# faasm/faabric

Measured on AMD Instinct MI355X. Metric: MPI_Allreduce GB/s + batch-exec msgs/sec, 8-rank world at 1/2/4/8 MI355X, higher is better.
Workload: dtype fp32; 1 GPU; model=faabric composite: 256MB fp32 allreduce + 1MB alltoall + kvtouch batch, global_batch=128, parallelism=mpi1, allreduce_bytes=268435456, pingpong_bytes=0, kv_bytes=4096, full=False, snapshot_bytes_per_rank=0, snapshot_dirty=random-scattered 25pct, random-byte region, gpu=True

## Files before the change

cpp/bindings/bindings_runtime.cpp:

```cpp
#include <pybind11/functional.h>
#include <pybind11/pybind11.h>
#include <pybind11/stl.h>

#include "faabricamd/endpoint.h"
#include "faabricamd/executor.h"
#include "faabricamd/flat.h"
#include "faabricamd/hipipc.h"
#include "faabricamd/planner.h"
#include "faabricamd/ptp.h"
#include "faabricamd/runner.h"
#include "faabricamd/scheduler.h"
#include "faabricamd/snapshot.h"
#include "faabricamd/state.h"
#include "faabricamd/util.h"
#include "faabricamd/utilextras.h"
#include "faabricamd/dirty.h"
#include <hip/hip_runtime.h>

namespace py = pybind11;
using namespace faabricamd;

namespace faabricamd {
void registerBenchFunctions();
std::map<std::string, std::vector<uint8_t>> benchLastOutputs();
// ... 826 lines not shown
            ok = dirty.size() == 16 && dirty[5] == 1 && dirty[12] == 1;
        }
        return py::bool_(ok);
    });

    m.def("_debug_runtime_sizes", [] {
        py::dict d;
        d["planner_app_results"] = Planner::get().debugAppResultsCount();
        d["planner_done_apps"] = Planner::get().debugDoneAppsCount();
        d["planner_in_flight"] = Planner::get().debugInFlightCount();
        d["broker_mappings"] = getPointToPointBroker().debugMappingsCount();
        d["broker_channels"] = getPointToPointBroker().debugChannelsCount();
        d["broker_send_seqs"] = getPointToPointBroker().debugSendSeqsCount();
        d["decision_cache"] = DecisionCache::get().size();
        return d;
    });
    m.def("_debug_dispatch_sizes", [] {
        py::dict d;
        d["idle_executors"] = Scheduler::get().debugIdleCount();
        d["planner_msg_index_apps"] = Planner::get().debugMsgIndexCount();
        d["planner_used_slots"] = Planner::get().debugUsedSlots();
        return d;
    });
    m.def("_debug_current_executor_id", [] {
        return ExecutorContext::get().getExecutor()->id;
    });
    m.def("_debug_set_message_result", [](const Message& msg) {
        auto copy = std::make_shared<Message>(msg);
        py::gil_scoped_release release;
        getPlannerClient().setMessageResult(copy);
    });
    m.def("_debug_kv_commit_stats", [] {
        KvCommitStats s = kvCommitStats();
        py::dict d;
        d["launches"] = s.launches;
        d["pages"] = s.pages;
        return d;
    });
    m.def("_debug_kv_sweep_bitmap",
          [](size_t nPages, const std::vector<uint64_t>& setBits) {
              size_t nWords = (nPages + 63) / 64;
              auto words = std::make_unique<std::atomic<uint64_t>[]>(
                std::max<size_t>(nWords, 1));
              for (size_t w = 0; w < nWords; w++) {
                  words[w].store(0);
              }
// ... 203 lines not shown
```

cpp/include/faabricamd/executor.h:

```cpp
#pragma once

#include <atomic>
#include <functional>
#include <memory>
#include <string>
#include <thread>
#include <vector>

#include "faabricamd/mailbox.h"
#include "faabricamd/messages.h"
#include "faabricamd/queue.h"
#include "faabricamd/dirty.h"
#include "faabricamd/snapshot.h"

namespace faabricamd {

class Executor;


class ExecutorContext
{
  public:
    static bool isSet();
    static void set(Executor* executor,
                    std::shared_ptr<BatchExecuteRequest> req,
                    int msgIdx);
    static void unset();
// ... 5 lines not shown
        return req;
    }
    Message& getMsg();
    int getMsgIdx() const { return msgIdx; }

  private:
    Executor* executor = nullptr;
    std::shared_ptr<BatchExecuteRequest> req;
    int msgIdx = 0;
};


using FaabricFunction = std::function<int32_t(Message&)>;

class FunctionRegistry
{
  public:
    static FunctionRegistry& get();
    void registerFunction(const std::string& user,
                          const std::string& function,
                          FaabricFunction fn);
    FaabricFunction* getFunction(const std::string& user,
                                 const std::string& function);
    void clear();

  private:
    std::mutex mx;
    std::map<std::string, FaabricFunction> functions;
};


struct ExecutorTask
{
    ExecutorTask() = default;
    ExecutorTask(int msgIdxIn, std::shared_ptr<BatchExecuteRequest> reqIn)
      : msgIdx(msgIdxIn)
      , req(std::move(reqIn))
    {}
    int msgIdx = 0;
    std::shared_ptr<BatchExecuteRequest> req;
    bool stop = false;
    bool single = false;
    int64_t enqueueNs = 0;
};

class Executor : public std::enable_shared_from_this<Executor>
{
  public:
    explicit Executor(Message& msg);
    virtual ~Executor();

    void executeTasks(const std::vector<int>& msgIdxs,
                      const std::shared_ptr<BatchExecuteRequest>& req);
    void executeSingleTask(int msgIdx,
                           const std::shared_ptr<BatchExecuteRequest>& req);

    std::vector<std::pair<int32_t, int32_t>> executeThreads(
      std::shared_ptr<BatchExecuteRequest> req,
      const std::vector<SnapshotMergeRegion>& mergeRegions);

    virtual int32_t executeTask(int threadPoolIdx,
                                int msgIdx,
                                std::shared_ptr<BatchExecuteRequest> req);

    virtual std::pair<uint8_t*, size_t> getMemoryView();
    virtual void setMemorySize(size_t newSize);
    void setDeviceMemorySize(size_t newSize);
    std::pair<uint8_t*, size_t> getDeviceMemoryView();
    bool hasDeviceArena() const { return deviceArena != nullptr; }
    virtual void restore(const std::string& snapshotKey);
    virtual void reset(Message& msg);
    virtual void flush();

    bool tryClaim();
    void claim();
    void releaseClaim();
    bool isClaimed() const { return claimed.load(); }
    using IdleExecutors = IdleList<std::shared_ptr<Executor>>;
// ... 73 lines not shown
```

cpp/include/faabricamd/mailbox.h:

```cpp
#pragma once

#include <atomic>
#include <climits>
#include <cstddef>
#include <cstdint>
#include <ctime>
#include <mutex>
#include <utility>
#include <vector>

#include <linux/futex.h>
#include <sys/syscall.h>
#include <unistd.h>

namespace faabricamd {

namespace detail {

inline void futexWait(std::atomic<uint32_t>* word,
                      uint32_t expected,
                      int timeoutMs)
{
    static_assert(sizeof(std::atomic<uint32_t>) == sizeof(uint32_t));
    struct timespec ts;
    struct timespec* tsp = nullptr;
    if (timeoutMs > 0) {
        ts.tv_sec = timeoutMs / 1000;
        ts.tv_nsec = (long)(timeoutMs % 1000) * 1000000L;
        tsp = &ts;
// ... 18 lines not shown
            0);
}

}

template<typename T, uint32_t SLOTS = 8>
class Mailbox
{
    static_assert(SLOTS >= 2 && (SLOTS & (SLOTS - 1)) == 0,
                  "SLOTS must be a power of two");

  public:
    Mailbox()
    {
        for (uint32_t i = 0; i < SLOTS; i++) {
            slots[i].seq.store(i, std::memory_order_relaxed);
        }
    }
    Mailbox(const Mailbox&) = delete;
    Mailbox& operator=(const Mailbox&) = delete;

    void post(T value)
    {
        uint32_t ticket = tail.fetch_add(1, std::memory_order_relaxed);
        Slot& s = slots[ticket & (SLOTS - 1)];
        uint32_t seen;
        while ((seen = s.seq.load(std::memory_order_acquire)) != ticket) {
            detail::futexWait(&s.seq, seen, 1);
        }
        s.value = std::move(value);
        s.seq.store(ticket + 1, std::memory_order_seq_cst);
        if (sleeping.load(std::memory_order_seq_cst) != 0) {
            detail::futexWake(&s.seq, INT_MAX);
        }
    }

    bool take(T& out, int timeoutMs)
    {
        Slot& s = slots[head & (SLOTS - 1)];
        uint32_t ready = head + 1;
        uint32_t seen = s.seq.load(std::memory_order_acquire);
        if (seen != ready) {
            struct timespec start;
            clock_gettime(CLOCK_MONOTONIC, &start);
            int leftMs = timeoutMs;
            while (true) {
                sleeping.store(1, std::memory_order_seq_cst);
                seen = s.seq.load(std::memory_order_seq_cst);
                if (seen != ready) {
                    detail::futexWait(&s.seq, seen, leftMs);
                    seen = s.seq.load(std::memory_order_acquire);
                }
                sleeping.store(0, std::memory_order_relaxed);
                if (seen == ready) {
                    break;
                }
                if (timeoutMs > 0) {
                    struct timespec now;
                    clock_gettime(CLOCK_MONOTONIC, &now);
                    int64_t goneMs =
                      (int64_t)(now.tv_sec - start.tv_sec) * 1000 +
                      (now.tv_nsec - start.tv_nsec) / 1000000;
                    if (goneMs >= timeoutMs) {
                        return false;
                    }
                    leftMs = (int)(timeoutMs - goneMs);
                }
            }
        }
        out = std::move(s.value);
        s.value = T();
        s.seq.store(head + SLOTS, std::memory_order_release);
        head++;
        return true;
    }

  private:
    struct alignas(64) Slot
    {
        std::atomic<uint32_t> seq{ 0 };
        T value{};
    };
    Slot slots[SLOTS];
    alignas(64) std::atomic<uint32_t> tail{ 0 };
    std::atomic<uint32_t> sleeping{ 0 };
    alignas(64) uint32_t head = 0;
};

template<typename T>
class IdleList
{
  public:
    void push(T value)
    {
        std::lock_guard<std::mutex> lock(mx);
        if (!closed) {
            entries.push_back(std::move(value));
        }
    }

    size_t popMany(size_t n, std::vector<T>& out)
    {
        std::lock_guard<std::mutex> lock(mx);
        size_t got = 0;
        while (got < n && !entries.empty()) {
            out.push_back(std::move(entries.back()));
            entries.pop_back();
            got++;
        }
        return got;
    }
// ... 53 lines not shown
```

cpp/include/faabricamd/scheduler.h:

```cpp
#pragma once

#include <memory>
#include <mutex>
#include <shared_mutex>
#include <unordered_map>
#include <vector>

#include "faabricamd/executor.h"
#include "faabricamd/messages.h"
#include "faabricamd/queue.h"
#include "faabricamd/transport.h"

namespace faabricamd {

enum class FunctionCalls : uint8_t
{
    ExecuteFunctions = 1,
    Flush = 2,
    SetMessageResult = 3,
    BatchDone = 4,
};

class Scheduler
{
// ... 3 lines not shown
    void executeBatch(std::shared_ptr<BatchExecuteRequest> req);

    HostResources getThisHostResources();
    void setThisHostResources(const HostResources& res);

    int reapStaleExecutors();
    void startReaper();
    void stopReaper();

    std::shared_ptr<PendingMigration> checkForMigrationOpportunities(
      Message& msg,
      int32_t overwriteNewGroupId = 0);

    void flushLocally();
    void shutdown();
    void reset();

    std::vector<Message> getRecordedMessages();
    void clearRecordedMessages();

    size_t getExecutorCount();
    size_t debugIdleCount();

  private:
    Scheduler();

    struct WarmPool
    {
        std::vector<std::shared_ptr<Executor>> list;
        std::shared_ptr<Executor::IdleExecutors> idle =
          std::make_shared<Executor::IdleExecutors>();
    };

    std::shared_ptr<Executor> claimExecutor(Message& msg);
    void claimExecutors(BatchExecuteRequest& req,
                        std::vector<std::shared_ptr<Executor>>& execs,
                        std::vector<std::string>& errors);
    std::shared_ptr<Executor> createExecutorLocked(WarmPool& pool,
                                                   Message& msg);

    std::shared_mutex schedMx;
    std::unordered_map<std::string, std::unique_ptr<WarmPool>> executors;
    HostResources overriddenResources;
    bool resourcesOverridden = false;

    std::vector<Message> recordedMessages;

    class ReaperThread;
    std::shared_ptr<ReaperThread> reaper;
};

bool functionCallServerRunning();

class FunctionCallServer : public MessageEndpointServer
{
  public:
    FunctionCallServer();
    ~FunctionCallServer() override;
// ... 30 lines not shown
```

cpp/include/faabricamd/state.h:

```cpp
#pragma once

#include <atomic>
#include <map>
#include <memory>
#include <mutex>
#include <string>
#include <vector>

#include "faabricamd/hipipc.h"
#include "faabricamd/messages.h"
#include "faabricamd/transport.h"

namespace faabricamd {

inline constexpr size_t STATE_STREAM_CHUNK_SIZE = 64 * 1024;

enum class StateCalls : uint8_t
{
    Pull = 1,
    Push = 2,
    Size = 3,
    Append = 4,
    ClearAppended = 5,
    PullAppended = 6,
    Delete = 7,
    PullIpc = 8,
    PushIpc = 9,
    Lock = 10,
// ... 135 lines not shown
    void forceClearAll(bool global);
    void syncAll();

    uint64_t acquireLock(const std::string& user,
                         const std::string& key,
                         int expiryMs);
    void releaseLock(const std::string& user,
                     const std::string& key,
                     uint64_t token);
    uint64_t acquireLockLocal(const std::string& user,
                              const std::string& key,
                              int expiryMs);
    bool releaseLockLocal(const std::string& user,
                          const std::string& key,
                          uint64_t token);

    void setMasterHost(const std::string& user,
                       const std::string& key,
                       const std::string& host);
    std::string getMasterHost(const std::string& user,
                              const std::string& key);

  private:
    std::mutex mx;
    std::map<std::string, std::shared_ptr<StateKeyValue>> kvMap;
    std::map<std::string, std::string> masterMap;

    std::mutex locksMx;
    std::map<std::string, std::pair<uint64_t, int64_t>> locks;
};

class StateServer : public MessageEndpointServer
{
  public:
    StateServer();
    void doAsyncRecv(uint8_t code,
                     const std::string& body,
                     uint32_t seq) override;
    std::string doSyncRecv(uint8_t code, const std::string& body) override;
};

class StateClient : public MessageEndpointClient
{
  public:
    explicit StateClient(const std::string& host);
    std::vector<uint8_t> pullChunk(const std::string& user,
                                   const std::string& key,
// ... 37 lines not shown
```

cpp/include/faabricamd/utilextras.h:

```cpp
#pragma once

#include <cstdint>
#include <string>
#include <vector>

namespace faabricamd {


struct DeltaConfig
{
    size_t pageSize = 4096;
    bool xorWithOld = true;
    bool compress = true;
    bool useZstd = true;

    static DeltaConfig parse(const std::string& s);
    std::string str() const;
};

std::vector<uint8_t> deltaEncode(const std::vector<uint8_t>& oldData,
                                 const std::vector<uint8_t>& newData,
                                 const DeltaConfig& conf = {});

std::vector<uint8_t> deltaApply(const std::vector<uint8_t>& oldData,
                                const std::vector<uint8_t>& delta);


void profStart(const std::string& name);
void profEnd(const std::string& name);
bool profEnabled();
int64_t profNowNs();
void profRecord(const char* name, double ms);
std::vector<std::pair<std::string, double>> profTotalsMs();
void profClear();
std::string profSummary();

#define PROF_START(name)                                                       \
    if (::faabricamd::profEnabled()) {                                         \
        ::faabricamd::profStart(#name);                                        \
    }
#define PROF_END(name)                                                         \
    if (::faabricamd::profEnabled()) {                                         \
        ::faabricamd::profEnd(#name);                                          \
    }

class ProfScope
{
  public:
    explicit ProfScope(const char* nameIn)
      : name(nameIn)
      , startNs(profEnabled() ? profNowNs() : 0)
    {}
    ~ProfScope()
    {
        if (startNs != 0) {
            profRecord(name, (double)(profNowNs() - startNs) / 1e6);
        }
    }
    ProfScope(const ProfScope&) = delete;
    ProfScope& operator=(const ProfScope&) = delete;

  private:
    const char* name;
    int64_t startNs;
};

void setUpCrashHandler();

int pinThreadToFreeCpu();
void unpinThisThread();

}
```

cpp/src/executor.cpp:

```cpp
#include "faabricamd/executor.h"
#include "faabricamd/utilextras.h"
#include "faabricamd/mpi.h"
#include "faabricamd/ops.h"
#include "faabricamd/planner.h"

#include <hip/hip_runtime.h>
#include "faabricamd/snapshot.h"
#include "faabricamd/util.h"

#include <algorithm>
#include <cstring>

namespace faabricamd {

void resultBatcherEnqueue(std::shared_ptr<Message> msg);


static thread_local std::shared_ptr<ExecutorContext> currentContext;

bool ExecutorContext::isSet()
{
    return currentContext != nullptr;
}

// ... 17 lines not shown
{
    if (!currentContext) {
        throw FaabricException("no executor context set");
    }
    return *currentContext;
}

Message& ExecutorContext::getMsg()
{
    return req->messages.at(msgIdx);
}


FunctionRegistry& FunctionRegistry::get()
{
    static FunctionRegistry reg;
    return reg;
}

void FunctionRegistry::registerFunction(const std::string& user,
                                        const std::string& function,
                                        FaabricFunction fn)
{
    std::lock_guard<std::mutex> lock(mx);
    functions[user + "/" + function] = std::move(fn);
}

FaabricFunction* FunctionRegistry::getFunction(const std::string& user,
                                               const std::string& function)
{
    std::lock_guard<std::mutex> lock(mx);
    auto it = functions.find(user + "/" + function);
    return it == functions.end() ? nullptr : &it->second;
}

void FunctionRegistry::clear()
{
    std::lock_guard<std::mutex> lock(mx);
    functions.clear();
}


Executor::Executor(Message& msg)
  : id(funcToString(msg.user, msg.function, 0) + "_" +
       std::to_string(generateGid()))
  , boundMsg(msg)
{
    threadPoolSize = std::min(getUsableCores(), 64);
    threadMailboxes.resize(threadPoolSize);
    threadPoolThreads.resize(threadPoolSize);
    poolThreadUp = std::make_unique<std::atomic<bool>[]>(threadPoolSize);
    for (int i = 0; i < threadPoolSize; i++) {
        poolThreadUp[i].store(false, std::memory_order_relaxed);
    }
    lastExecMs = getGlobalClockEpochMillis();
}

void Executor::cleanupForkSnapshot()
{
    if (lastForkSnapshotKey.empty()) {
        return;
    }
// ... 101 lines not shown
void Executor::ensurePoolThreadLocked(int poolIdx)
{
    if (threadPoolThreads[poolIdx].joinable()) {
        return;
    }
    if (!threadMailboxes[poolIdx]) {
        threadMailboxes[poolIdx] = std::make_unique<TaskMailbox>();
    }
    threadPoolThreads[poolIdx] =
      std::thread([this, poolIdx] { threadPoolThread(poolIdx); });
    poolThreadUp[poolIdx].store(true, std::memory_order_release);
}

void Executor::postTask(int poolIdx, ExecutorTask&& task)
{
    task.enqueueNs = profEnabled() ? profNowNs() : 0;
    threadMailboxes[poolIdx]->post(std::move(task));
}

void Executor::executeSingleTask(
  int msgIdx,
  const std::shared_ptr<BatchExecuteRequest>& req)
{
    if (req->type == BatchExecuteType::THREADS ||
        !req->snapshotKey.empty() ||
        !req->messages.at(msgIdx).snapshotKey.empty() ||
        threadPoolSize == 0) {
        executeTasks({ msgIdx }, req);
        return;
    }
    lastExecMs = getGlobalClockEpochMillis();
    if (!poolThreadUp[0].load(std::memory_order_acquire)) {
        std::lock_guard<std::mutex> lock(threadsMx);
        ensurePoolThreadLocked(0);
    }
    ExecutorTask task(msgIdx, req);
    task.single = true;
    postTask(0, std::move(task));
}

void Executor::executeTasks(const std::vector<int>& msgIdxs,
                            const std::shared_ptr<BatchExecuteRequest>& req)
{
    lastExecMs = getGlobalClockEpochMillis();
    batchCounter = std::make_shared<std::atomic<int>>((int)msgIdxs.size());

    if (!req->snapshotKey.empty()) {
        restore(req->snapshotKey);
    } else if (!req->messages.empty() &&
               !req->messages[msgIdxs[0]].snapshotKey.empty() &&
               req->type != BatchExecuteType::THREADS) {
        const std::string& key = req->messages[msgIdxs[0]].snapshotKey;
        restore(key);
        if (startsWith(key, "migration_")) {
            SnapshotRegistry::get().deleteSnapshot(key);
            DeviceSnapshotRegistry::get().deleteSnapshot(key);
        }
    }

    if (req->type == BatchExecuteType::THREADS &&
        !req->snapshotKey.empty()) {
// ... 128 lines not shown
        hipError_t err = hipMemcpy(deviceArena,
                                   dsnap->data(),
                                   dsnap->size(),
                                   hipMemcpyDeviceToDevice);
        if (err != hipSuccess ||
            hipStreamSynchronize(nullptr) != hipSuccess) {
            throw FaabricException("device snapshot merge-back failed");
        }
    } else {
        snap->writeQueuedDiffs();
        auto [memBase2, memSize2] = getMemoryView();
        snap->mapToMemory(memBase2, memSize2);
        snap->clearMergeRegions();
    }
    return results;
}

int32_t Executor::executeTask(int threadPoolIdx,
                              int msgIdx,
                              std::shared_ptr<BatchExecuteRequest> req)
{
    (void)threadPoolIdx;
    Message& msg = req->messages.at(msgIdx);
    FaabricFunction* fn =
      FunctionRegistry::get().getFunction(msg.user, msg.function);
    if (fn == nullptr) {
        throw FaabricException("function not registered: " + msg.user + "/" +
                               msg.function);
    }
    return (*fn)(msg);
}

std::pair<uint8_t*, size_t> Executor::getMemoryView()
{
    return { dummyMemory.data(), dummyMemory.size() };
}

void Executor::setMemorySize(size_t newSize)
{
    dummyMemory.resize(newSize);
}

void Executor::restore(const std::string& snapshotKey)
{
    const auto& conf = getSystemConfig();
    int64_t deadline = getGlobalClockEpochMillis() + conf.boundTimeout;
    while (true) {
        if (DeviceSnapshotRegistry::get().snapshotExists(snapshotKey)) {
            auto dsnap =
              DeviceSnapshotRegistry::get().getSnapshot(snapshotKey);
            if (deviceArenaSize < dsnap->size()) {
                setDeviceMemorySize(dsnap->size());
            }
// ... 36 lines not shown
void Executor::setThreadResult(Message& msg,
                               int32_t returnValue,
                               const std::string& key,
                               const std::vector<SnapshotDiffMsg>& diffs)
{
    (void)key;
    (void)diffs;
    msg.returnValue = returnValue;
}

void Executor::threadPoolThread(int poolIdx)
{
    const auto& conf = getSystemConfig();
    TaskMailbox& mailbox = *threadMailboxes[poolIdx];
    while (true) {
        ExecutorTask task;
        if (!mailbox.take(task, conf.boundTimeout)) {
            continue;
        }
        if (task.stop) {
            break;
        }
        if (task.enqueueNs != 0) {
            profRecord("exec_wake",
                       (double)(profNowNs() - task.enqueueNs) / 1e6);
        }

        Message& msg = task.req->messages.at(task.msgIdx);
        int32_t returnValue = 0;
        ExecutorContext::set(this, task.req, task.msgIdx);
        try {
            PROF_START(exec_task)
            returnValue = executeTask(poolIdx, task.msgIdx, task.req);
            PROF_END(exec_task)
            if (msg.isMpi && msg.recordExecGraph &&
                MpiWorldRegistry::get().worldExists(msg.mpiWorldId)) {
                auto counts = MpiWorldRegistry::get()
                                .getWorld(msg.mpiWorldId)
                                .getMsgCountDetails(msg.mpiRank);
                for (const auto& [k, v] : counts) {
                    msg.intExecGraphDetails[k] = v;
                }
            }
        } catch (const FunctionMigratedException&) {
            FAM_DEBUG("task %d migrated", msg.id);
            returnValue = MIGRATED_FUNCTION_RETURN_VALUE;
        } catch (const FunctionFrozenException&) {
            FAM_DEBUG("task %d frozen", msg.id);
// ... 259 lines not shown
```

cpp/src/scheduler.cpp:

```cpp
#include "faabricamd/scheduler.h"
#include "faabricamd/utilextras.h"

#include <atomic>
#include <thread>
#include <functional>
#include <condition_variable>
#include "faabricamd/planner.h"
#include "faabricamd/ptp.h"
#include "faabricamd/util.h"
#include "faabricamd/wire.h"

#include <hip/hip_runtime.h>

namespace faabricamd {

static int getNumGpus()
{
    static int n = []() {
        const auto& conf = getSystemConfig();
        if (conf.overrideGpuCount >= 0) {
            return conf.overrideGpuCount;
        }
        if (!conf.useGpu) {
            return 0;
// ... 23 lines not shown

HostResources Scheduler::getThisHostResources()
{
    {
        std::unique_lock<std::shared_mutex> lock(schedMx);
        if (resourcesOverridden) {
            return overriddenResources;
        }
    }
    HostResources res;
    int nGpus = getNumGpus();
    res.slots = nGpus > 0 ? nGpus : getUsableCores();
    res.usedSlots = 0;
    return res;
}

void Scheduler::setThisHostResources(const HostResources& res)
{
    std::unique_lock<std::shared_mutex> lock(schedMx);
    overriddenResources = res;
    resourcesOverridden = true;
}

void Scheduler::executeBatch(std::shared_ptr<BatchExecuteRequest> req)
{
    if (req->messages.empty()) {
        return;
    }
    PROF_START(sched_execute_batch)
    bool isThreads = req->type == BatchExecuteType::THREADS;

    if (isTestMode()) {
        std::unique_lock<std::shared_mutex> lock(schedMx);
        for (const auto& msg : req->messages) {
            recordedMessages.push_back(msg);
        }
    }

    if (isThreads) {
        auto exec = claimExecutor(req->messages[0]);
        std::vector<int> idxs(req->messages.size());
        for (size_t i = 0; i < idxs.size(); i++) {
            idxs[i] = (int)i;
        }
        exec->executeTasks(idxs, req);
    } else {
        size_t n = req->messages.size();
        std::vector<std::shared_ptr<Executor>> execs;
        std::vector<std::string> claimErrors;
        PROF_START(dispatch_claim)
        claimExecutors(*req, execs, claimErrors);
        PROF_END(dispatch_claim)

        PROF_START(dispatch_enqueue)
        for (size_t i = 0; i < n; i++) {
            try {
                if (!execs[i]) {
                    throw FaabricException(claimErrors[i]);
                }
                execs[i]->executeSingleTask((int)i, req);
            } catch (const std::exception& e) {
                FAM_ERROR("claiming executor failed: %s", e.what());
                if (execs[i]) {
                    execs[i]->releaseClaim();
                }
                auto msg = std::make_shared<Message>(req->messages[i]);
                msg->returnValue = 1;
                msg->executedHost = getSystemConfig().endpointHost;
                msg->outputData = std::string("executor claim failed: ") +
                                  e.what();
                getPlannerClient().setMessageResult(msg);
            }
        }
        PROF_END(dispatch_enqueue)
    }
    PROF_END(sched_execute_batch)
}

static std::shared_ptr<Executor> popIdleClaimed(
  Executor::IdleExecutors& idle)
{
    std::shared_ptr<Executor> e;
    while (idle.pop(e)) {
        if (e->tryClaim()) {
            return e;
        }
    }
    return nullptr;
}

std::shared_ptr<Executor> Scheduler::createExecutorLocked(WarmPool& pool,
                                                          Message& msg)
{
    auto exec = getExecutorFactory()->createExecutor(msg);
    exec->claim();
// ... 14 lines not shown
    std::string key = msg.user + "/" + msg.function;

    {
        std::shared_lock<std::shared_mutex> rlock(schedMx);
        auto it = executors.find(key);
        if (it != executors.end()) {
            if (auto e = popIdleClaimed(*it->second->idle)) {
                return e;
            }
        }
    }

    std::unique_lock<std::shared_mutex> lock(schedMx);
    auto& poolPtr = executors[key];
    if (!poolPtr) {
        poolPtr = std::make_unique<WarmPool>();
    }
    if (auto e = popIdleClaimed(*poolPtr->idle)) {
        return e;
    }
    return createExecutorLocked(*poolPtr, msg);
}

void Scheduler::claimExecutors(
  BatchExecuteRequest& req,
  std::vector<std::shared_ptr<Executor>>& execs,
  std::vector<std::string>& errors)
{
    size_t n = req.messages.size();
    execs.assign(n, nullptr);
    errors.assign(n, std::string());

    const Message& first = req.messages[0];
    bool oneFunction = true;
    for (size_t i = 1; i < n && oneFunction; i++) {
        oneFunction = req.messages[i].function == first.function &&
                      req.messages[i].user == first.user;
    }
    if (!oneFunction) {
        for (size_t i = 0; i < n; i++) {
            try {
                execs[i] = claimExecutor(req.messages[i]);
            } catch (const std::exception& e) {
                errors[i] = e.what();
            }
        }
        return;
    }

    std::string key = first.user + "/" + first.function;
    std::vector<std::shared_ptr<Executor>> popped;
    popped.reserve(n);
    size_t got = 0;
    auto takeIdle = [&](Executor::IdleExecutors& idle) {
        while (got < n) {
            popped.clear();
            if (idle.popMany(n - got, popped) == 0) {
                return;
            }
            for (auto& e : popped) {
                if (e->tryClaim()) {
                    execs[got++] = std::move(e);
                }
            }
        }
    };
    {
        std::shared_lock<std::shared_mutex> rlock(schedMx);
        auto it = executors.find(key);
        if (it != executors.end()) {
            takeIdle(*it->second->idle);
        }
    }
    if (got == n) {
        return;
    }

    std::unique_lock<std::shared_mutex> lock(schedMx);
    auto& poolPtr = executors[key];
    if (!poolPtr) {
        poolPtr = std::make_unique<WarmPool>();
    }
    takeIdle(*poolPtr->idle);
    poolPtr->list.reserve(poolPtr->list.size() + (n - got));
    for (; got < n; got++) {
        try {
            execs[got] = createExecutorLocked(*poolPtr, req.messages[got]);
        } catch (const std::exception& e) {
            errors[got] = e.what();
        }
    }
}

int Scheduler::reapStaleExecutors()
{
    std::unique_lock<std::shared_mutex> lock(schedMx);
    const auto& conf = getSystemConfig();
    int reaped = 0;
    for (auto& [key, pool] : executors) {
        auto& list = pool->list;
        for (auto it = list.begin(); it != list.end();) {
            auto& exec = *it;
            if (exec->getMillisSinceLastExec() > conf.boundTimeout &&
                exec->tryClaim()) {
                pool->idle->remove(exec);
                exec->shutdown();
                it = list.erase(it);
                reaped++;
            } else {
                ++it;
            }
        }
    }
    return reaped;
// ... 332 lines not shown
```

cpp/src/state.cpp:

```cpp
#include "faabricamd/state.h"
#include "faabricamd/ops.h"
#include "faabricamd/ptp.h"
#include "faabricamd/util.h"
#include "faabricamd/utilextras.h"

#include <hip/hip_runtime.h>

#include <algorithm>
#include <cstring>

namespace faabricamd {

static std::string kvKeyOf(const std::string& user, const std::string& key)
{
    return user + "/" + key;
}

static std::mutex gStripeMx[StateKeyValue::KV_STRIPES];

static std::mutex gCommitMx;
static hipStream_t gCommitStream = nullptr;
static uint32_t* gCommitList = nullptr;
static uint32_t* gCommitListDev = nullptr;
static size_t gCommitListCap = 0;
// ... 911 lines not shown
    appendedValues.clear();
}


State& State::get()
{
    static State st;
    return st;
}

static std::string defaultMasterHost()
{
    auto& conf = getSystemConfig();
    if (conf.stateMode == "planner") {
        return conf.plannerHost;
    }
    return conf.endpointHost;
}

std::shared_ptr<StateKeyValue> State::getKV(const std::string& user,
                                            const std::string& key,
                                            size_t size)
{
    std::lock_guard<std::mutex> lock(mx);
    std::string k = kvKeyOf(user, key);
    auto it = kvMap.find(k);
    if (it != kvMap.end()) {
        return it->second;
    }
    std::string master;
    auto mIt = masterMap.find(k);
    if (mIt != masterMap.end()) {
        master = mIt->second;
    } else {
        master = defaultMasterHost();
        masterMap[k] = master;
    }
    auto kv = std::make_shared<StateKeyValue>(user, key, size, master);
    kvMap[k] = kv;
    return kv;
}

std::shared_ptr<StateKeyValue> State::getKVDevice(const std::string& user,
                                                  const std::string& key,
                                                  size_t size,
                                                  int device)
{
    std::lock_guard<std::mutex> lock(mx);
    std::string k = kvKeyOf(user, key);
    auto it = kvMap.find(k);
    if (it != kvMap.end()) {
        return it->second;
    }
    std::string master;
    auto mIt = masterMap.find(k);
    if (mIt != masterMap.end()) {
        master = mIt->second;
    } else {
        master = defaultMasterHost();
        masterMap[k] = master;
    }
    auto kv = std::make_shared<StateKeyValue>(
      user, key, size, master, true, device);
    kvMap[k] = kv;
    return kv;
}

std::shared_ptr<StateKeyValue> State::getKV(const std::string& user,
                                            const std::string& key)
{
    std::lock_guard<std::mutex> lock(mx);
    auto it = kvMap.find(kvKeyOf(user, key));
    if (it == kvMap.end()) {
        throw FaabricException("state key not found: " +
                               kvKeyOf(user, key));
    }
    return it->second;
}

size_t State::getStateSize(const std::string& user, const std::string& key)
{
    {
        std::lock_guard<std::mutex> lock(mx);
        auto it = kvMap.find(kvKeyOf(user, key));
        if (it != kvMap.end()) {
            return it->second->size();
        }
    }
    std::string master = getMasterHost(user, key);
    if (!master.empty() && master != getSystemConfig().endpointHost) {
        return getStateClient(master)->stateSize(user, key);
    }
    return 0;
}

void State::deleteKV(const std::string& user, const std::string& key)
{
    std::string master;
    {
        std::lock_guard<std::mutex> lock(mx);
        auto mIt = masterMap.find(kvKeyOf(user, key));
        master = mIt == masterMap.end() ? "" : mIt->second;
    }
    if (!master.empty() && master != getSystemConfig().endpointHost) {
        getStateClient(master)->deleteKV(user, key);
    }
    deleteKVLocally(user, key);
}

void State::deleteKVLocally(const std::string& user, const std::string& key)
{
    std::lock_guard<std::mutex> lock(mx);
    kvMap.erase(kvKeyOf(user, key));
    masterMap.erase(kvKeyOf(user, key));
}

size_t State::getKVCount()
{
    std::lock_guard<std::mutex> lock(mx);
    return kvMap.size();
}

void State::syncAll()
{
    std::vector<std::shared_ptr<StateKeyValue>> kvs;
    {
        std::lock_guard<std::mutex> lock(mx);
        kvs.reserve(kvMap.size());
        for (auto& [k, kv] : kvMap) {
            kvs.push_back(kv);
        }
    }
    PROF_START(kv_sync)
    try {
        StateKeyValue::syncMany(kvs);
    } catch (...) {
        PROF_END(kv_sync)
        throw;
    }
    PROF_END(kv_sync)
}

void State::forceClearAll(bool global)
{
    (void)global;
    std::lock_guard<std::mutex> lock(mx);
    kvMap.clear();
    masterMap.clear();
}

uint64_t State::acquireLockLocal(const std::string& user,
                                 const std::string& key,
                                 int expiryMs)
{
    std::lock_guard<std::mutex> lock(locksMx);
    std::string k = kvKeyOf(user, key);
    int64_t now = getEpochMicros() / 1000;
    auto it = locks.find(k);
    if (it != locks.end() && it->second.second > now) {
        return 0;
    }
    uint64_t token = ((uint64_t)generateGid() << 32) | generateGid();
    if (token == 0) {
        token = 1;
    }
    locks[k] = { token, now + expiryMs };
    return token;
}

// ... 24 lines not shown
    }
    return getStateClient(owner)->acquireLock(user, key, expiryMs);
}

void State::releaseLock(const std::string& user,
                        const std::string& key,
                        uint64_t token)
{
    std::string owner = getMasterHost(user, key);
    if (owner.empty()) {
        owner = defaultMasterHost();
    }
    if (owner == getSystemConfig().endpointHost) {
        releaseLockLocal(user, key, token);
        return;
    }
    getStateClient(owner)->releaseLock(user, key, token);
}

void State::setMasterHost(const std::string& user,
                          const std::string& key,
                          const std::string& host)
{
    std::lock_guard<std::mutex> lock(mx);
    masterMap[kvKeyOf(user, key)] = host;
}

std::string State::getMasterHost(const std::string& user,
                                 const std::string& key)
{
    std::lock_guard<std::mutex> lock(mx);
    auto it = masterMap.find(kvKeyOf(user, key));
    return it == masterMap.end() ? "" : it->second;
}


StateServer::StateServer()
  : MessageEndpointServer(STATE_ASYNC_PORT, STATE_SYNC_PORT, "state")
{}

void StateServer::doAsyncRecv(uint8_t code,
                              const std::string& body,
                              uint32_t seq)
{
    (void)code;
    (void)body;
    (void)seq;
    FAM_ERROR("state server has no async calls");
}

std::string StateServer::doSyncRecv(uint8_t code, const std::string& body)
{
    auto& st = State::get();
    switch ((StateCalls)code) {
// ... 272 lines not shown
```

cpp/src/utilextras.cpp:

```cpp
#include "faabricamd/utilextras.h"
#include "faabricamd/util.h"

#include <atomic>
#include <chrono>
#include <csignal>
#include <cstring>
#include <execinfo.h>
#include <map>
#include <mutex>
#include <pthread.h>
#include <sched.h>
#include <sstream>
#include <thread>
#include <zlib.h>

namespace faabricamd {


enum DeltaCmd : uint8_t
{
    DELTA_TOTAL_SIZE = 1,
    DELTA_XOR_PAGE = 2,
    DELTA_RAW_RANGE = 3,
    DELTA_COMPRESSED = 4,
    DELTA_COMPRESSED_ZSTD = 5,
    DELTA_END = 0xff,
};

extern "C" {
size_t ZSTD_compressBound(size_t srcSize);
size_t ZSTD_compress(void* dst,
                     size_t dstCapacity,
                     const void* src,
                     size_t srcSize,
                     int level);
// ... 188 lines not shown
                for (uint64_t i = 0; i < len; i++) {
                    out[off + i] ^= cmds[p + i];
                }
                p += len;
                break;
            }
            case DELTA_RAW_RANGE: {
                uint64_t off = getU64(cmds.data() + p);
                uint64_t len = getU64(cmds.data() + p + 8);
                p += 16;
                std::memcpy(out.data() + off, cmds.data() + p, len);
                p += len;
                break;
            }
            default:
                throw FaabricException("bad delta command");
        }
    }
    return out;
}


namespace {
struct ProfState
{
    std::mutex mx;
    std::map<std::string, double> totalsMs;
    std::map<std::string, int64_t> counts;
};
ProfState& profState()
{
    static ProfState st;
    return st;
}
thread_local std::map<std::string, std::chrono::steady_clock::time_point>
  profStarts;
}

bool profEnabled()
{
    static const bool v = getEnvVarInt("FAABRIC_PROF", 0) != 0;
    return v;
}

int64_t profNowNs()
{
    return std::chrono::duration_cast<std::chrono::nanoseconds>(
             std::chrono::steady_clock::now().time_since_epoch())
      .count();
}

void profRecord(const char* name, double ms)
{
    if (!profEnabled()) {
        return;
    }
    auto& st = profState();
    std::lock_guard<std::mutex> lock(st.mx);
    st.totalsMs[name] += ms;
    st.counts[name] += 1;
}

void profStart(const std::string& name)
{
    if (!profEnabled()) {
        return;
    }
    profStarts[name] = std::chrono::steady_clock::now();
}

void profEnd(const std::string& name)
{
    if (!profEnabled()) {
        return;
    }
    auto it = profStarts.find(name);
    if (it == profStarts.end()) {
        return;
    }
    double ms = std::chrono::duration<double, std::milli>(
                  std::chrono::steady_clock::now() - it->second)
                  .count();
    profStarts.erase(it);
    auto& st = profState();
    std::lock_guard<std::mutex> lock(st.mx);
    st.totalsMs[name] += ms;
    st.counts[name] += 1;
}

std::vector<std::pair<std::string, double>> profTotalsMs()
{
    auto& st = profState();
    std::lock_guard<std::mutex> lock(st.mx);
    return { st.totalsMs.begin(), st.totalsMs.end() };
}

void profClear()
{
    auto& st = profState();
    std::lock_guard<std::mutex> lock(st.mx);
    st.totalsMs.clear();
    st.counts.clear();
}

std::string profSummary()
{
    auto& st = profState();
    std::lock_guard<std::mutex> lock(st.mx);
    std::ostringstream out;
    out << "--- PROF totals ---\n";
    for (const auto& [name, ms] : st.totalsMs) {
        out << name << ": " << ms << " ms (" << st.counts[name]
            << " calls)\n";
    }
    return out.str();
}


static void crashHandler(int sig)
{
    void* frames[64];
    int n = backtrace(frames, 64);
    fprintf(stderr, "--- crash: signal %d (%s) ---\n", sig,
            strsignal(sig));
    backtrace_symbols_fd(frames, n, 2);
    signal(sig, SIG_DFL);
    raise(sig);
}

void setUpCrashHandler()
{
    signal(SIGABRT, crashHandler);
    signal(SIGILL, crashHandler);
    signal(SIGFPE, crashHandler);
}
// ... 42 lines not shown
```

Measured before the change: 227,400 msgs/sec.

## Add relay-wake dispatch, thread-local function cache, shared mutexes and per-thread profiler

Adds an opt-in wake-relay dispatch path in which the scheduler posts tasks to executors without waking them, and each woken executor then wakes the next, spreading futex wake cost across threads. It caches function lookups per thread, keyed on a registry generation counter. The registry and state maps switch to shared_mutex, and the profiler moves to lock-free per-thread tables. The relay path is off by default (chains=0), so the default-path changes are the lookup cache and the lock changes. These add complexity and new debug hooks, with some risk of races in the relay path.

```diff
diff --git a/cpp/bindings/bindings_runtime.cpp b/cpp/bindings/bindings_runtime.cpp
--- a/cpp/bindings/bindings_runtime.cpp
+++ b/cpp/bindings/bindings_runtime.cpp
@@ -872,6 +872,19 @@
         d["planner_used_slots"] = Planner::get().debugUsedSlots();
         return d;
     });
+    m.def("_debug_set_dispatch_chains", &Scheduler::debugSetDispatchChains);
+    m.def("_debug_dispatch_chains", &Scheduler::dispatchChains);
+    m.def("_debug_relayed_batches", &Scheduler::debugRelayedBatches);
+    m.def("_debug_fail_next_claim_at", &Scheduler::debugFailNextClaimAt);
+    m.def("_debug_prof_set_enabled", &profSetEnabled);
+    m.def("_debug_prof_enabled", &profEnabled);
+    m.def("_debug_prof_record",
+          [](const std::string& name, double ms, int times) {
+              py::gil_scoped_release release;
+              for (int i = 0; i < times; i++) {
+                  profRecord(name.c_str(), ms);
+              }
+          });
     m.def("_debug_current_executor_id", [] {
         return ExecutorContext::get().getExecutor()->id;
     });
diff --git a/cpp/include/faabricamd/executor.h b/cpp/include/faabricamd/executor.h
--- a/cpp/include/faabricamd/executor.h
+++ b/cpp/include/faabricamd/executor.h
@@ -2,7 +2,10 @@
 
 #include <atomic>
 #include <functional>
+#include <map>
 #include <memory>
+#include <mutex>
+#include <shared_mutex>
 #include <string>
 #include <thread>
 #include <vector>
@@ -54,13 +57,33 @@
                           FaabricFunction fn);
     FaabricFunction* getFunction(const std::string& user,
                                  const std::string& function);
+    FaabricFunction* getFunction(const std::string& user,
+                                 const std::string& function,
+                                 uint64_t& generationOut);
+    uint64_t generation() const
+    {
+        return gen.load(std::memory_order_acquire);
+    }
     void clear();
 
   private:
-    std::mutex mx;
+    std::shared_mutex mx;
+    std::atomic<uint64_t> gen{ 1 };
     std::map<std::string, FaabricFunction> functions;
 };
 
+
+struct WakeRelay
+{
+    explicit WakeRelay(std::vector<std::shared_ptr<Executor>> execsIn)
+      : execs(std::move(execsIn))
+      , cursor((uint32_t)execs.size())
+    {}
+    std::vector<std::shared_ptr<Executor>> execs;
+    WakeCursor cursor;
+
+    bool step();
+};
 
 struct ExecutorTask
 {
@@ -74,6 +97,7 @@
     bool stop = false;
     bool single = false;
     int64_t enqueueNs = 0;
+    std::shared_ptr<WakeRelay> relay;
 };
 
 class Executor : public std::enable_shared_from_this<Executor>
@@ -86,6 +110,12 @@
                       const std::shared_ptr<BatchExecuteRequest>& req);
     void executeSingleTask(int msgIdx,
                            const std::shared_ptr<BatchExecuteRequest>& req);
+    static bool singleTaskFastPath(const BatchExecuteRequest& req,
+                                   int msgIdx);
+    void postSingleTaskQuiet(int msgIdx,
+                             const std::shared_ptr<BatchExecuteRequest>& req,
+                             std::shared_ptr<WakeRelay> relay);
+    bool wakeSingleTaskThread();
 
     std::vector<std::pair<int32_t, int32_t>> executeThreads(
       std::shared_ptr<BatchExecuteRequest> req,
diff --git a/cpp/include/faabricamd/mailbox.h b/cpp/include/faabricamd/mailbox.h
--- a/cpp/include/faabricamd/mailbox.h
+++ b/cpp/include/faabricamd/mailbox.h
@@ -5,6 +5,7 @@
 #include <cstddef>
 #include <cstdint>
 #include <ctime>
+#include <memory>
 #include <mutex>
 #include <utility>
 #include <vector>
@@ -69,6 +70,12 @@
 
     void post(T value)
     {
+        postQuiet(std::move(value));
+        wakeIfSleeping();
+    }
+
+    void postQuiet(T value)
+    {
         uint32_t ticket = tail.fetch_add(1, std::memory_order_relaxed);
         Slot& s = slots[ticket & (SLOTS - 1)];
         uint32_t seen;
@@ -77,9 +84,16 @@
         }
         s.value = std::move(value);
         s.seq.store(ticket + 1, std::memory_order_seq_cst);
-        if (sleeping.load(std::memory_order_seq_cst) != 0) {
-            detail::futexWake(&s.seq, INT_MAX);
-        }
+    }
+
+    bool wakeIfSleeping()
+    {
+        uint32_t where = sleeping.load(std::memory_order_seq_cst);
+        if (where == 0) {
+            return false;
+        }
+        detail::futexWake(&slots[(where - 1) & (SLOTS - 1)].seq, INT_MAX);
+        return true;
     }
 
     bool take(T& out, int timeoutMs)
@@ -92,7 +106,8 @@
             clock_gettime(CLOCK_MONOTONIC, &start);
             int leftMs = timeoutMs;
             while (true) {
-                sleeping.store(1, std::memory_order_seq_cst);
+                sleeping.store((head & (SLOTS - 1)) + 1,
+                               std::memory_order_seq_cst);
                 seen = s.seq.load(std::memory_order_seq_cst);
                 if (seen != ready) {
                     detail::futexWait(&s.seq, seen, leftMs);
@@ -134,6 +149,68 @@
     alignas(64) uint32_t head = 0;
 };
 
+class WakeCursor
+{
+  public:
+    explicit WakeCursor(uint32_t nIn)
+      : n(nIn)
+      , taken(new std::atomic<uint8_t>[nIn ? nIn : 1])
+    {
+        for (uint32_t i = 0; i < n; i++) {
+            taken[i].store(0, std::memory_order_relaxed);
+        }
+    }
+    WakeCursor(const WakeCursor&) = delete;
+    WakeCursor& operator=(const WakeCursor&) = delete;
+
+    void open() { cursor.store(0, std::memory_order_seq_cst); }
+
+    bool claim(uint32_t& pos)
+    {
+        if (cursor.load(std::memory_order_seq_cst) >= n) {
+            return false;
+        }
+        uint32_t p = cursor.fetch_add(1, std::memory_order_seq_cst);
+        if (p >= n) {
+            return false;
+        }
+        pos = p;
+        return true;
+    }
+
+    void markTaken(uint32_t pos)
+    {
+        taken[pos].store(1, std::memory_order_seq_cst);
+    }
+
+    bool isTaken(uint32_t pos) const
+    {
+        return taken[pos].load(std::memory_order_seq_cst) != 0;
+    }
+
+    template<typename Wake>
+    uint32_t relay(Wake&& wake)
+    {
+        uint32_t claimed = 0;
+        uint32_t pos;
+        while (claim(pos)) {
+            claimed++;
+            if (!isTaken(pos) && wake(pos)) {
+                break;
+            }
+        }
+        return claimed;
+    }
+
+    uint32_t size() const { return n; }
+
+  private:
+    static constexpr uint32_t CLOSED = UINT32_MAX / 2;
+    const uint32_t n;
+    std::unique_ptr<std::atomic<uint8_t>[]> taken;
+    alignas(64) std::atomic<uint32_t> cursor{ CLOSED };
+};
+
 template<typename T>
 class IdleList
 {
diff --git a/cpp/include/faabricamd/scheduler.h b/cpp/include/faabricamd/scheduler.h
--- a/cpp/include/faabricamd/scheduler.h
+++ b/cpp/include/faabricamd/scheduler.h
@@ -49,6 +49,11 @@
     size_t getExecutorCount();
     size_t debugIdleCount();
 
+    static int dispatchChains();
+    static void debugSetDispatchChains(int chains);
+    static uint64_t debugRelayedBatches();
+    static void debugFailNextClaimAt(int msgIdx);
+
   private:
     Scheduler();
 
@@ -60,7 +65,7 @@
     };
 
     std::shared_ptr<Executor> claimExecutor(Message& msg);
-    void claimExecutors(BatchExecuteRequest& req,
+    bool claimExecutors(BatchExecuteRequest& req,
                         std::vector<std::shared_ptr<Executor>>& execs,
                         std::vector<std::string>& errors);
     std::shared_ptr<Executor> createExecutorLocked(WarmPool& pool,
diff --git a/cpp/include/faabricamd/state.h b/cpp/include/faabricamd/state.h
--- a/cpp/include/faabricamd/state.h
+++ b/cpp/include/faabricamd/state.h
@@ -4,6 +4,7 @@
 #include <map>
 #include <memory>
 #include <mutex>
+#include <shared_mutex>
 #include <string>
 #include <vector>
 
@@ -185,7 +186,7 @@
                               const std::string& key);
 
   private:
-    std::mutex mx;
+    std::shared_mutex mx;
     std::map<std::string, std::shared_ptr<StateKeyValue>> kvMap;
     std::map<std::string, std::string> masterMap;
 
diff --git a/cpp/include/faabricamd/utilextras.h b/cpp/include/faabricamd/utilextras.h
--- a/cpp/include/faabricamd/utilextras.h
+++ b/cpp/include/faabricamd/utilextras.h
@@ -29,8 +29,10 @@
 void profStart(const std::string& name);
 void profEnd(const std::string& name);
 bool profEnabled();
+void profSetEnabled(bool on);
 int64_t profNowNs();
 void profRecord(const char* name, double ms);
+void profRecordNs(const char* name, int64_t ns);
 std::vector<std::pair<std::string, double>> profTotalsMs();
 void profClear();
 std::string profSummary();
@@ -54,7 +56,7 @@
     ~ProfScope()
     {
         if (startNs != 0) {
-            profRecord(name, (double)(profNowNs() - startNs) / 1e6);
+            profRecordNs(name, profNowNs() - startNs);
         }
     }
     ProfScope(const ProfScope&) = delete;
diff --git a/cpp/src/executor.cpp b/cpp/src/executor.cpp
--- a/cpp/src/executor.cpp
+++ b/cpp/src/executor.cpp
@@ -63,22 +63,37 @@
                                         const std::string& function,
                                         FaabricFunction fn)
 {
-    std::lock_guard<std::mutex> lock(mx);
-    functions[user + "/" + function] = std::move(fn);
+    std::string key = user + "/" + function;
+    std::unique_lock<std::shared_mutex> lock(mx);
+    functions[key] = std::move(fn);
+    gen.fetch_add(1, std::memory_order_acq_rel);
 }
 
 FaabricFunction* FunctionRegistry::getFunction(const std::string& user,
                                                const std::string& function)
 {
-    std::lock_guard<std::mutex> lock(mx);
-    auto it = functions.find(user + "/" + function);
+    std::string key = user + "/" + function;
+    std::shared_lock<std::shared_mutex> lock(mx);
+    auto it = functions.find(key);
     return it == functions.end() ? nullptr : &it->second;
 }
 
+FaabricFunction* FunctionRegistry::getFunction(const std::string& user,
+                                               const std::string& function,
+                                               uint64_t& generationOut)
+{
+    std::string key = user + "/" + function;
+    std::shared_lock<std::shared_mutex> lock(mx);
+    generationOut = gen.load(std::memory_order_acquire);
+    auto it = functions.find(key);
+    return it == functions.end() ? nullptr : &it->second;
+}
+
 void FunctionRegistry::clear()
 {
-    std::lock_guard<std::mutex> lock(mx);
+    std::unique_lock<std::shared_mutex> lock(mx);
     functions.clear();
+    gen.fetch_add(1, std::memory_order_acq_rel);
 }
 
 
@@ -226,13 +241,26 @@
   int msgIdx,
   const std::shared_ptr<BatchExecuteRequest>& req)
 {
-    if (req->type == BatchExecuteType::THREADS ||
-        !req->snapshotKey.empty() ||
-        !req->messages.at(msgIdx).snapshotKey.empty() ||
-        threadPoolSize == 0) {
+    if (!singleTaskFastPath(*req, msgIdx) || threadPoolSize == 0) {
         executeTasks({ msgIdx }, req);
         return;
     }
+    postSingleTaskQuiet(msgIdx, req, nullptr);
+    wakeSingleTaskThread();
+}
+
+bool Executor::singleTaskFastPath(const BatchExecuteRequest& req, int msgIdx)
+{
+    return req.type != BatchExecuteType::THREADS &&
+           req.snapshotKey.empty() &&
+           req.messages.at(msgIdx).snapshotKey.empty();
+}
+
+void Executor::postSingleTaskQuiet(
+  int msgIdx,
+  const std::shared_ptr<BatchExecuteRequest>& req,
+  std::shared_ptr<WakeRelay> relay)
+{
     lastExecMs = getGlobalClockEpochMillis();
     if (!poolThreadUp[0].load(std::memory_order_acquire)) {
         std::lock_guard<std::mutex> lock(threadsMx);
@@ -240,7 +268,26 @@
     }
     ExecutorTask task(msgIdx, req);
     task.single = true;
-    postTask(0, std::move(task));
+    task.relay = std::move(relay);
+    task.enqueueNs = profEnabled() ? profNowNs() : 0;
+    threadMailboxes[0]->postQuiet(std::move(task));
+}
+
+bool Executor::wakeSingleTaskThread()
+{
+    return threadMailboxes[0]->wakeIfSleeping();
+}
+
+bool WakeRelay::step()
+{
+    int64_t t0 = profEnabled() ? profNowNs() : 0;
+    uint32_t claimed = cursor.relay([this](uint32_t pos) {
+        return execs[pos] && execs[pos]->wakeSingleTaskThread();
+    });
+    if (t0 != 0 && claimed > 0) {
+        profRecordNs("dispatch_wake", profNowNs() - t0);
+    }
+    return claimed > 0;
 }
 
 void Executor::executeTasks(const std::vector<int>& msgIdxs,
@@ -415,13 +462,27 @@
 {
     (void)threadPoolIdx;
     Message& msg = req->messages.at(msgIdx);
-    FaabricFunction* fn =
-      FunctionRegistry::get().getFunction(msg.user, msg.function);
-    if (fn == nullptr) {
+    struct Resolved
+    {
+        uint64_t generation = 0;
+        std::string user;
+        std::string function;
+        FaabricFunction* fn = nullptr;
+    };
+    static thread_local Resolved cached;
+    auto& registry = FunctionRegistry::get();
+    if (cached.generation != registry.generation() ||
+        cached.function != msg.function || cached.user != msg.user) {
+        cached.fn =
+          registry.getFunction(msg.user, msg.function, cached.generation);
+        cached.user = msg.user;
+        cached.function = msg.function;
+    }
+    if (cached.fn == nullptr) {
         throw FaabricException("function not registered: " + msg.user + "/" +
                                msg.function);
     }
-    return (*fn)(msg);
+    return (*cached.fn)(msg);
 }
 
 std::pair<uint8_t*, size_t> Executor::getMemoryView()
@@ -504,8 +565,12 @@
             break;
         }
         if (task.enqueueNs != 0) {
-            profRecord("exec_wake",
-                       (double)(profNowNs() - task.enqueueNs) / 1e6);
+            profRecordNs("exec_wake", profNowNs() - task.enqueueNs);
+        }
+        if (task.relay) {
+            task.relay->cursor.markTaken((uint32_t)task.msgIdx);
+            task.relay->step();
+            task.relay.reset();
         }
 
         Message& msg = task.req->messages.at(task.msgIdx);
diff --git a/cpp/src/scheduler.cpp b/cpp/src/scheduler.cpp
--- a/cpp/src/scheduler.cpp
+++ b/cpp/src/scheduler.cpp
@@ -69,6 +69,39 @@
     resourcesOverridden = true;
 }
 
+static constexpr int DEFAULT_DISPATCH_CHAINS = 0;
+static std::atomic<int> dispatchChainsOverride{ -1 };
+static std::atomic<int> failNextClaimAt{ -1 };
+static std::atomic<uint64_t> relayedBatches{ 0 };
+
+uint64_t Scheduler::debugRelayedBatches()
+{
+    return relayedBatches.load(std::memory_order_relaxed);
+}
+
+int Scheduler::dispatchChains()
+{
+    int forced = dispatchChainsOverride.load(std::memory_order_relaxed);
+    if (forced >= 0) {
+        return forced;
+    }
+    static const int fromEnv = std::max(
+      0, getEnvVarInt("FAABRIC_DISPATCH_CHAINS", DEFAULT_DISPATCH_CHAINS));
+    return fromEnv;
+}
+
+void Scheduler::debugSetDispatchChains(int chains)
+{
+    dispatchChainsOverride.store(chains < 0 ? -1 : chains,
+                                 std::memory_order_relaxed);
+}
+
+void Scheduler::debugFailNextClaimAt(int msgIdx)
+{
+    failNextClaimAt.store(msgIdx < 0 ? -1 : msgIdx,
+                          std::memory_order_relaxed);
+}
+
 void Scheduler::executeBatch(std::shared_ptr<BatchExecuteRequest> req)
 {
     if (req->messages.empty()) {
@@ -96,20 +129,57 @@
         std::vector<std::shared_ptr<Executor>> execs;
         std::vector<std::string> claimErrors;
         PROF_START(dispatch_claim)
-        claimExecutors(*req, execs, claimErrors);
+        bool oneFunction = claimExecutors(*req, execs, claimErrors);
         PROF_END(dispatch_claim)
-
+        int failAt = failNextClaimAt.load(std::memory_order_relaxed);
+        if (failAt >= 0 && (size_t)failAt < n &&
+            failNextClaimAt.compare_exchange_strong(failAt, -1)) {
+            if (execs[failAt]) {
+                execs[failAt]->releaseClaim();
+                execs[failAt] = nullptr;
+            }
+            claimErrors[failAt] = "injected claim failure";
+        }
+
+        int chains = dispatchChains();
+        bool relayed = chains > 0 && n > 1 && oneFunction;
+        for (size_t i = 0; i < n && relayed; i++) {
+            relayed = Executor::singleTaskFastPath(*req, (int)i);
+        }
+        std::shared_ptr<WakeRelay> relay;
+        if (relayed) {
+            relay = std::make_shared<WakeRelay>(std::move(execs));
+            relayedBatches.fetch_add(1, std::memory_order_relaxed);
+        }
+        auto& handOff = relay ? relay->execs : execs;
+        bool timed = profEnabled();
+        int64_t postNs = 0;
+        int64_t wakeNs = 0;
+        int64_t loopStartNs = timed ? profNowNs() : 0;
         PROF_START(dispatch_enqueue)
         for (size_t i = 0; i < n; i++) {
             try {
-                if (!execs[i]) {
+                if (!handOff[i]) {
                     throw FaabricException(claimErrors[i]);
                 }
-                execs[i]->executeSingleTask((int)i, req);
+                if (relay) {
+                    handOff[i]->postSingleTaskQuiet((int)i, req, relay);
+                } else if (timed &&
+                           Executor::singleTaskFastPath(*req, (int)i)) {
+                    int64_t t0 = profNowNs();
+                    handOff[i]->postSingleTaskQuiet((int)i, req, nullptr);
+                    int64_t t1 = profNowNs();
+                    bool woke = handOff[i]->wakeSingleTaskThread();
+                    postNs += t1 - t0;
+                    wakeNs += woke ? profNowNs() - t1 : 0;
+                } else {
+                    handOff[i]->executeSingleTask((int)i, req);
+                }
             } catch (const std::exception& e) {
                 FAM_ERROR("claiming executor failed: %s", e.what());
-                if (execs[i]) {
-                    execs[i]->releaseClaim();
+                if (handOff[i]) {
+                    handOff[i]->releaseClaim();
+                    handOff[i] = nullptr;
                 }
                 auto msg = std::make_shared<Message>(req->messages[i]);
                 msg->returnValue = 1;
@@ -118,6 +188,17 @@
                                   e.what();
                 getPlannerClient().setMessageResult(msg);
             }
+        }
+        if (relay) {
+            if (timed) {
+                profRecordNs("dispatch_post", profNowNs() - loopStartNs);
+            }
+            relay->cursor.open();
+            for (int c = 0; c < chains && relay->step(); c++) {
+            }
+        } else if (timed) {
+            profRecordNs("dispatch_post", postNs);
+            profRecordNs("dispatch_wake", wakeNs);
         }
         PROF_END(dispatch_enqueue)
     }
@@ -178,7 +259,7 @@
     return createExecutorLocked(*poolPtr, msg);
 }
 
-void Scheduler::claimExecutors(
+bool Scheduler::claimExecutors(
   BatchExecuteRequest& req,
   std::vector<std::shared_ptr<Executor>>& execs,
   std::vector<std::string>& errors)
@@ -201,7 +282,7 @@
                 errors[i] = e.what();
             }
         }
-        return;
+        return false;
     }
 
     std::string key = first.user + "/" + first.function;
@@ -229,7 +310,7 @@
         }
     }
     if (got == n) {
-        return;
+        return true;
     }
 
     std::unique_lock<std::shared_mutex> lock(schedMx);
@@ -246,6 +327,7 @@
             errors[got] = e.what();
         }
     }
+    return true;
 }
 
 int Scheduler::reapStaleExecutors()
diff --git a/cpp/src/state.cpp b/cpp/src/state.cpp
--- a/cpp/src/state.cpp
+++ b/cpp/src/state.cpp
@@ -957,8 +957,15 @@
                                             const std::string& key,
                                             size_t size)
 {
-    std::lock_guard<std::mutex> lock(mx);
     std::string k = kvKeyOf(user, key);
+    {
+        std::shared_lock<std::shared_mutex> rlock(mx);
+        auto hit = kvMap.find(k);
+        if (hit != kvMap.end()) {
+            return hit->second;
+        }
+    }
+    std::unique_lock<std::shared_mutex> lock(mx);
     auto it = kvMap.find(k);
     if (it != kvMap.end()) {
         return it->second;
@@ -981,8 +988,15 @@
                                                   size_t size,
                                                   int device)
 {
-    std::lock_guard<std::mutex> lock(mx);
     std::string k = kvKeyOf(user, key);
+    {
+        std::shared_lock<std::shared_mutex> rlock(mx);
+        auto hit = kvMap.find(k);
+        if (hit != kvMap.end()) {
+            return hit->second;
+        }
+    }
+    std::unique_lock<std::shared_mutex> lock(mx);
     auto it = kvMap.find(k);
     if (it != kvMap.end()) {
         return it->second;
@@ -1004,11 +1018,11 @@
 std::shared_ptr<StateKeyValue> State::getKV(const std::string& user,
                                             const std::string& key)
 {
-    std::lock_guard<std::mutex> lock(mx);
-    auto it = kvMap.find(kvKeyOf(user, key));
+    std::string k = kvKeyOf(user, key);
+    std::shared_lock<std::shared_mutex> lock(mx);
+    auto it = kvMap.find(k);
     if (it == kvMap.end()) {
-        throw FaabricException("state key not found: " +
-                               kvKeyOf(user, key));
+        throw FaabricException("state key not found: " + k);
     }
     return it->second;
 }
@@ -1016,7 +1030,7 @@
 size_t State::getStateSize(const std::string& user, const std::string& key)
 {
     {
-        std::lock_guard<std::mutex> lock(mx);
+        std::unique_lock<std::shared_mutex> lock(mx);
         auto it = kvMap.find(kvKeyOf(user, key));
         if (it != kvMap.end()) {
             return it->second->size();
@@ -1033,7 +1047,7 @@
 {
     std::string master;
     {
-        std::lock_guard<std::mutex> lock(mx);
+        std::unique_lock<std::shared_mutex> lock(mx);
         auto mIt = masterMap.find(kvKeyOf(user, key));
         master = mIt == masterMap.end() ? "" : mIt->second;
     }
@@ -1045,14 +1059,14 @@
 
 void State::deleteKVLocally(const std::string& user, const std::string& key)
 {
-    std::lock_guard<std::mutex> lock(mx);
+    std::unique_lock<std::shared_mutex> lock(mx);
     kvMap.erase(kvKeyOf(user, key));
     masterMap.erase(kvKeyOf(user, key));
 }
 
 size_t State::getKVCount()
 {
-    std::lock_guard<std::mutex> lock(mx);
+    std::unique_lock<std::shared_mutex> lock(mx);
     return kvMap.size();
 }
 
@@ -1060,7 +1074,7 @@
 {
     std::vector<std::shared_ptr<StateKeyValue>> kvs;
     {
-        std::lock_guard<std::mutex> lock(mx);
+        std::unique_lock<std::shared_mutex> lock(mx);
         kvs.reserve(kvMap.size());
         for (auto& [k, kv] : kvMap) {
             kvs.push_back(kv);
@@ -1079,7 +1093,7 @@
 void State::forceClearAll(bool global)
 {
     (void)global;
-    std::lock_guard<std::mutex> lock(mx);
+    std::unique_lock<std::shared_mutex> lock(mx);
     kvMap.clear();
     masterMap.clear();
 }
@@ -1150,14 +1164,14 @@
                           const std::string& key,
                           const std::string& host)
 {
-    std::lock_guard<std::mutex> lock(mx);
+    std::unique_lock<std::shared_mutex> lock(mx);
     masterMap[kvKeyOf(user, key)] = host;
 }
 
 std::string State::getMasterHost(const std::string& user,
                                  const std::string& key)
 {
-    std::lock_guard<std::mutex> lock(mx);
+    std::unique_lock<std::shared_mutex> lock(mx);
     auto it = masterMap.find(kvKeyOf(user, key));
     return it == masterMap.end() ? "" : it->second;
 }
diff --git a/cpp/src/utilextras.cpp b/cpp/src/utilextras.cpp
--- a/cpp/src/utilextras.cpp
+++ b/cpp/src/utilextras.cpp
@@ -1,8 +1,10 @@
 #include "faabricamd/utilextras.h"
 #include "faabricamd/util.h"
 
+#include <algorithm>
 #include <atomic>
 #include <chrono>
+#include <cmath>
 #include <csignal>
 #include <cstring>
 #include <execinfo.h>
@@ -11,6 +13,7 @@
 #include <pthread.h>
 #include <sched.h>
 #include <sstream>
+#include <string_view>
 #include <thread>
 #include <zlib.h>
 
@@ -245,25 +248,150 @@
 
 
 namespace {
-struct ProfState
+
+struct ProfNode
+{
+    explicit ProfNode(std::string nameIn)
+      : name(std::move(nameIn))
+    {}
+    const std::string name;
+    std::atomic<int64_t> totalNs{ 0 };
+    std::atomic<int64_t> calls{ 0 };
+    std::atomic<ProfNode*> next{ nullptr };
+};
+
+struct ProfTable
+{
+    std::atomic<ProfNode*> head{ nullptr };
+    ProfNode* tail = nullptr;
+    std::map<std::string, ProfNode*, std::less<>> index;
+
+    ~ProfTable()
+    {
+        ProfNode* n = head.load(std::memory_order_relaxed);
+        while (n != nullptr) {
+            ProfNode* next = n->next.load(std::memory_order_relaxed);
+            delete n;
+            n = next;
+        }
+    }
+
+    ProfNode* node(std::string_view name)
+    {
+        auto it = index.find(name);
+        if (it != index.end()) {
+            return it->second;
+        }
+        auto* n = new ProfNode(std::string(name));
+        if (tail == nullptr) {
+            head.store(n, std::memory_order_release);
+        } else {
+            tail->next.store(n, std::memory_order_release);
+        }
+        tail = n;
+        index.emplace(n->name, n);
+        return n;
+    }
+};
+
+struct ProfRegistry
 {
     std::mutex mx;
-    std::map<std::string, double> totalsMs;
-    std::map<std::string, int64_t> counts;
+    std::vector<ProfTable*> live;
+    std::map<std::string, std::pair<int64_t, int64_t>> retired;
 };
-ProfState& profState()
-{
-    static ProfState st;
-    return st;
-}
+
+ProfRegistry& profRegistry()
+{
+    static ProfRegistry* reg = new ProfRegistry();
+    return *reg;
+}
+
+struct ProfThreadSlot
+{
+    ProfTable* table = nullptr;
+
+    ProfTable& get()
+    {
+        if (table == nullptr) {
+            table = new ProfTable();
+            auto& reg = profRegistry();
+            std::lock_guard<std::mutex> lock(reg.mx);
+            reg.live.push_back(table);
+        }
+        return *table;
+    }
+
+    ~ProfThreadSlot()
+    {
+        if (table == nullptr) {
+            return;
+        }
+        auto& reg = profRegistry();
+        {
+            std::lock_guard<std::mutex> lock(reg.mx);
+            for (ProfNode* n = table->head.load(std::memory_order_acquire);
+                 n != nullptr;
+                 n = n->next.load(std::memory_order_acquire)) {
+                auto& r = reg.retired[n->name];
+                r.first += n->totalNs.load(std::memory_order_relaxed);
+                r.second += n->calls.load(std::memory_order_relaxed);
+            }
+            reg.live.erase(
+              std::find(reg.live.begin(), reg.live.end(), table));
+        }
+        delete table;
+        table = nullptr;
+    }
+};
+
+thread_local ProfThreadSlot profSlot;
 thread_local std::map<std::string, std::chrono::steady_clock::time_point>
   profStarts;
+
+std::atomic<bool>& profFlag()
+{
+    static std::atomic<bool> v{ getEnvVarInt("FAABRIC_PROF", 0) != 0 };
+    return v;
+}
+
+void profAdd(std::string_view name, int64_t ns)
+{
+    ProfNode* n = profSlot.get().node(name);
+    n->totalNs.fetch_add(ns, std::memory_order_relaxed);
+    n->calls.fetch_add(1, std::memory_order_relaxed);
+}
+
+std::map<std::string, std::pair<int64_t, int64_t>> profMergeLocked(
+  ProfRegistry& reg)
+{
+    auto merged = reg.retired;
+    for (ProfTable* t : reg.live) {
+        for (ProfNode* n = t->head.load(std::memory_order_acquire);
+             n != nullptr;
+             n = n->next.load(std::memory_order_acquire)) {
+            int64_t calls = n->calls.load(std::memory_order_relaxed);
+            if (calls == 0) {
+                continue;
+            }
+            auto& m = merged[n->name];
+            m.first += n->totalNs.load(std::memory_order_relaxed);
+            m.second += calls;
+        }
+    }
+    return merged;
+}
+
 }
 
 bool profEnabled()
 {
-    static const bool v = getEnvVarInt("FAABRIC_PROF", 0) != 0;
-    return v;
+    return profFlag().load(std::memory_order_relaxed);
+}
+
+void profSetEnabled(bool on)
+{
+    profFlag().store(on, std::memory_order_relaxed);
 }
 
 int64_t profNowNs()
@@ -273,15 +401,20 @@
       .count();
 }
 
-void profRecord(const char* name, double ms)
+void profRecordNs(const char* name, int64_t ns)
 {
     if (!profEnabled()) {
         return;
     }
-    auto& st = profState();
-    std::lock_guard<std::mutex> lock(st.mx);
-    st.totalsMs[name] += ms;
-    st.counts[name] += 1;
+    profAdd(name, ns);
+}
+
+void profRecord(const char* name, double ms)
+{
+    if (!profEnabled()) {
+        return;
+    }
+    profAdd(name, std::llround(ms * 1e6));
 }
 
 void profStart(const std::string& name)
@@ -301,39 +434,47 @@
     if (it == profStarts.end()) {
         return;
     }
-    double ms = std::chrono::duration<double, std::milli>(
-                  std::chrono::steady_clock::now() - it->second)
-                  .count();
+    int64_t ns = std::chrono::duration_cast<std::chrono::nanoseconds>(
+                   std::chrono::steady_clock::now() - it->second)
+                   .count();
     profStarts.erase(it);
-    auto& st = profState();
-    std::lock_guard<std::mutex> lock(st.mx);
-    st.totalsMs[name] += ms;
-    st.counts[name] += 1;
+    profAdd(name, ns);
 }
 
 std::vector<std::pair<std::string, double>> profTotalsMs()
 {
-    auto& st = profState();
-    std::lock_guard<std::mutex> lock(st.mx);
-    return { st.totalsMs.begin(), st.totalsMs.end() };
+    auto& reg = profRegistry();
+    std::lock_guard<std::mutex> lock(reg.mx);
+    std::vector<std::pair<std::string, double>> out;
+    for (const auto& [name, v] : profMergeLocked(reg)) {
+        out.emplace_back(name, (double)v.first / 1e6);
+    }
+    return out;
 }
 
 void profClear()
 {
-    auto& st = profState();
-    std::lock_guard<std::mutex> lock(st.mx);
-    st.totalsMs.clear();
-    st.counts.clear();
+    auto& reg = profRegistry();
+    std::lock_guard<std::mutex> lock(reg.mx);
+    reg.retired.clear();
+    for (ProfTable* t : reg.live) {
+        for (ProfNode* n = t->head.load(std::memory_order_acquire);
+             n != nullptr;
+             n = n->next.load(std::memory_order_acquire)) {
+            n->totalNs.store(0, std::memory_order_relaxed);
+            n->calls.store(0, std::memory_order_relaxed);
+        }
+    }
 }
 
 std::string profSummary()
 {
-    auto& st = profState();
-    std::lock_guard<std::mutex> lock(st.mx);
+    auto& reg = profRegistry();
+    std::lock_guard<std::mutex> lock(reg.mx);
     std::ostringstream out;
     out << "--- PROF totals ---\n";
-    for (const auto& [name, ms] : st.totalsMs) {
-        out << name << ": " << ms << " ms (" << st.counts[name]
+    for (const auto& [name, v] : profMergeLocked(reg)) {
+        out << name << ": " << (double)v.first / 1e6 << " ms (" << v.second
             << " calls)\n";
     }
     return out.str();
```

New measurement: 197,200 msgs/sec. -13.3%, worse.
